# ExaScience/bpmf

Hardware: AMD Instinct MI355X
Metric: user+item column samples/sec per Gibbs iter; test RMSE vs reference (higher is better)
Workload: dtype f64

## Files before the change

### bpmf_amd/csrc/kernels.h

```cpp
#pragma once
#include <hip/hip_runtime.h>
#include <stdint.h>

#include "philox.h"
#include "args.h"

namespace bpmf {

typedef double d4 __attribute__((ext_vector_type(4)));

__device__ __forceinline__ d4 mfma16(double a, double b, d4 c)
{
    return __builtin_amdgcn_mfma_f64_16x16x4f64(a, b, c, 0, 0, 0);
}

__device__ __forceinline__ double mfma44(double a, double b, double c)
{
    return __builtin_amdgcn_mfma_f64_4x4x4f64(a, b, c, 0, 0, 0);
}

template <int K>
struct Rot44 {
    static constexpr int NT = K / 16;
    __host__ __device__ static constexpr int nrot(int TI, int TJ) { return TI == TJ ? 3 : 4; }
    __host__ __device__ static constexpr int aoff(int TI, int TJ)
    {
        int n = 0;
        for (int a = 0; a < NT; ++a)
            for (int b = a; b < NT; ++b) {
                if (a == TI && b == TJ) return n;
                n += nrot(a, b);
            }
        return n;
    }
    static constexpr int NACC = aoff(NT - 1, NT - 1) + 3;
};

template <int D>
__device__ __forceinline__ double quad_rot(double x)
{
    constexpr int CTRL = 0x120 + (16 - 4 * D);
    const long long v = __builtin_bit_cast(long long, x);
    const int lo = __builtin_amdgcn_update_dpp(0, (int)v, CTRL, 0xF, 0xF, true);
    const int hi = __builtin_amdgcn_update_dpp(0, (int)(v >> 32), CTRL, 0xF, 0xF, true);
    return __builtin_bit_cast(double, ((long long)hi << 32) | (unsigned int)lo);
}

template <int K>
__device__ __forceinline__ void rot44_contract(const double (&yy)[K / 16], double (&C)[Rot44<K>::NACC])
{
    using G = Rot44<K>;
    constexpr int NT = K / 16;
    double rot[NT][3];
#pragma unroll
    for (int t = 0; t < NT; ++t) {
        rot[t][0] = yy[t];
        rot[t][1] = quad_rot<1>(yy[t]);
        rot[t][2] = quad_rot<2>(yy[t]);
    }
#pragma unroll
    for (int TI = 0; TI < NT; ++TI)
#pragma unroll
        for (int TJ = TI; TJ < NT; ++TJ)
#pragma unroll
            for (int d = 0; d < G::nrot(TI, TJ); ++d) {
                if (d < 3) C[G::aoff(TI, TJ) + d] = mfma44(yy[TI], rot[TJ][d], C[G::aoff(TI, TJ) + d]);
                else C[G::aoff(TI, TJ) + d] = mfma44(rot[TI][1], yy[TJ], C[G::aoff(TI, TJ) + d]);
            }
}

template <int K, typename Sink>
__device__ __forceinline__ void rot44_images(const double (&C)[Rot44<K>::NACC], double *buf0, double *buf1, int lane, Sink &&sink)
{
    using G = Rot44<K>;
    constexpr int NT = G::NT;
    const int i = lane >> 4, b = (lane >> 2) & 3, j = lane & 3;
    int tix = 0;
#pragma unroll
    for (int TI = 0; TI < NT; ++TI)
#pragma unroll
        for (int TJ = TI; TJ < NT; ++TJ, ++tix) {
            double *img = (tix & 1) ? buf1 : buf0;
#pragma unroll
            for (int d = 0; d < G::nrot(TI, TJ); ++d) {
                const int row = d < 3 ? 4 * b + i : 4 * ((b + 1) & 3) + i, col = d < 3 ? 4 * ((b + d) & 3) + j : 4 * b + j;
                const double v = C[G::aoff(TI, TJ) + d];
                img[row * 16 + col] = v;
                if (TI == TJ && d > 0) img[col * 16 + row] = v;
            }
            __syncthreads();
#pragma unroll
            for (int m = 0; m < 4; ++m) sink(tix, TI, TJ, m, img[(4 * m + i) * 16 + (lane & 15)]);
            __syncthreads();
        }
}

__device__ __forceinline__ double rsqrt_nr(double d)
{
    const double y0 = __builtin_amdgcn_rsq(d);
    const double e = fma(-d, y0 * y0, 1.0);
    const double q = e * fma(0.375, e, 0.5);
    return fma(y0, q, y0);
}

__device__ __forceinline__ double gbcast(double v, int base_bytes, int off)
{
    const int lo = __builtin_amdgcn_ds_bpermute(base_bytes + 4 * off, __double2loint(v));
    const int hi = __builtin_amdgcn_ds_bpermute(base_bytes + 4 * off, __double2hiint(v));
    return __hiloint2double(hi, lo);
}

__device__ __forceinline__ double bcast(double v, int src)
{
    const int lo = __builtin_amdgcn_readlane(__double2loint(v), src);
    const int hi = __builtin_amdgcn_readlane(__double2hiint(v), src);
    return __hiloint2double(hi, lo);
}


__device__ __forceinline__ double polar_r2(double x, double y)
{
#pragma clang fp contract(off)
    return x * x + y * y;
}

__device__ __forceinline__ uint32_t sample_counter(int64_t idx, int ktrue, uint32_t iter_plus_1)
{
    return (uint32_t)((uint64_t)(idx + 1) * (uint64_t)ktrue * (uint64_t)iter_plus_1);
}

#define BPMF_RLX_SYSTEM_ __ATOMIC_RELAXED, __HIP_MEMORY_SCOPE_SYSTEM
enum { BPMF_TMO_GATE = 1, BPMF_TMO_PARAMS = 2, BPMF_TMO_STATS = 3 };
__device__ __forceinline__ void flag_timeout(unsigned long long *tmo, unsigned long long what)
{
    if (tmo) __hip_atomic_store(tmo, what, BPMF_RLX_SYSTEM_);
}

__device__ __forceinline__ void wait_params(const SampleArgs &a)
{
    if (a.gate_flag == nullptr) return;
    const unsigned long long t0 = wall_clock64();
    const unsigned long long limit = a.wait_ticks + (a.wait_ticks >> 1);
    while ((unsigned)__builtin_amdgcn_readfirstlane((int)__hip_atomic_load(a.gate_flag, __ATOMIC_RELAXED, __HIP_MEMORY_SCOPE_AGENT)) != a.gate_want) {
        __builtin_amdgcn_s_sleep(8);
        if (wall_clock64() - t0 > limit) {
            if (threadIdx.x == 0) flag_timeout(a.tmo, BPMF_TMO_PARAMS);
            break;
        }
    }
    asm volatile("" ::: "memory");
}

#ifndef BPMF_PROFILING
#define BPMF_PROFILING 0
#endif
constexpr bool kProfiling = BPMF_PROFILING != 0;
__device__ __forceinline__ uint32_t ablate_bits(const SampleArgs &a)
{
    if constexpr (kProfiling) return a.ablate;
    else return 0u;
}

__device__ __forceinline__ void stamp(const SampleArgs &a, int w, int slot)
{
    if constexpr (!kProfiling) {
        __builtin_amdgcn_sched_barrier(0);
        return;
    }
    if (a.stamps == nullptr || threadIdx.x != 0) return;
    const int probe = (w == 0) ? 0 : ((w == a.nwork / 2) ? 1 : -1);
    if (probe >= 0 && slot < 64) a.stamps[probe * 64 + slot] = wall_clock64();
}

__device__ __forceinline__ int rank_below(unsigned long long m)
{
    return (int)__builtin_amdgcn_mbcnt_hi((unsigned)(m >> 32), __builtin_amdgcn_mbcnt_lo((unsigned)m, 0u));
}

template <int NMAX>
__device__ __forceinline__ void draw_normals(uint32_t counter, int n, double *out_lds, int lane, int pad_to = 0)
{
    for (int i = n + lane; i < pad_to; i += 64) out_lds[i] = 0.0;
    int produced = 0;
    uint32_t base = 0;
    while (produced < n) {
        const Philox4 b = stream_block(counter, base + (uint32_t)lane);
        const double x = 2.0 * canonical53(b.w[3], b.w[2]) - 1.0;
        const double y = 2.0 * canonical53(b.w[1], b.w[0]) - 1.0;
        const double r2 = polar_r2(x, y);
        const bool acc = !(r2 > 1.0 || r2 == 0.0);
        const unsigned long long m = __ballot(acc);
        const int rank = produced + rank_below(m);
        if (acc && rank < n) {
            out_lds[rank] = y * polar_mult(r2);
        }
        produced += __popcll(m);
        base += 64u;
    }
}

template <int NMAX>
__device__ __forceinline__ void draw_normals_deferred(uint32_t counter, int n, double *out_lds, double *r2_lds, int lane, int pad_to = 0)
{
    for (int i = n + lane; i < pad_to; i += 64) out_lds[i] = 0.0;
    int produced = 0;
    uint32_t base = 0;
    while (produced < n) {
        const Philox4 b = stream_block(counter, base + (uint32_t)lane);
        const double x = 2.0 * canonical53(b.w[3], b.w[2]) - 1.0;
        const double y = 2.0 * canonical53(b.w[1], b.w[0]) - 1.0;
        const double r2 = polar_r2(x, y);
        const bool acc = !(r2 > 1.0 || r2 == 0.0);
        const unsigned long long m = __ballot(acc);
        const int rank = produced + rank_below(m);
        if (acc && rank < n) { out_lds[rank] = y; r2_lds[rank] = r2; }
        produced += __popcll(m);
        base += 64u;
    }
    for (int i = lane; i < n; i += 64) {
        const double r2 = r2_lds[i];
        out_lds[i] = out_lds[i] * polar_mult(r2);
    }
}

template <int NMAX>
__device__ __forceinline__ void draw_normals_pair(uint32_t counterA, uint32_t counterB, int n, double *outA, double *outB,
                                                  double *r2A, double *r2B, int lane, int pad_to = 0)
{
    for (int i = n + lane; i < pad_to; i += 64) { outA[i] = 0.0; outB[i] = 0.0; }
    auto attempt = [&](uint32_t counter, uint32_t block, double &y, double &r2) -> bool {
        const Philox4 b = stream_block(counter, block);
        const double x = 2.0 * canonical53(b.w[3], b.w[2]) - 1.0;
        y = 2.0 * canonical53(b.w[1], b.w[0]) - 1.0;
        r2 = polar_r2(x, y);
        return !(r2 > 1.0 || r2 == 0.0);
    };
    int prodA, prodB;
    {
        double y, r2;
        bool acc = attempt(counterA, (uint32_t)lane, y, r2);
        unsigned long long m = __ballot(acc);
        int rank = rank_below(m);
        if (acc && rank < n) { outA[rank] = y; r2A[rank] = r2; }
        prodA = __popcll(m);
        acc = attempt(counterB, (uint32_t)lane, y, r2);
        m = __ballot(acc);
        rank = rank_below(m);
        if (acc && rank < n) { outB[rank] = y; r2B[rank] = r2; }
        prodB = __popcll(m);
    }
    const bool hi = lane >= 32;
    const int l32 = lane & 31;
    uint32_t base = 64u;
    while (prodA < n || prodB < n) {
        double y, r2;
        const bool acc = attempt(hi ? counterB : counterA, base + (uint32_t)l32, y, r2);
        const unsigned long long m = __ballot(acc);
        const unsigned mA = (unsigned)m, mB = (unsigned)(m >> 32);
        const int rank = hi ? prodB + (int)__builtin_amdgcn_mbcnt_hi(mB, 0u) : prodA + (int)__builtin_amdgcn_mbcnt_lo(mA, 0u);
        if (acc && rank < n) { (hi ? outB : outA)[rank] = y; (hi ? r2B : r2A)[rank] = r2; }
        prodA += __popc(mA); prodB += __popc(mB);
        base += 32u;
    }
    for (int i = lane; i < n; i += 64) {
        const double ra = r2A[i], rb = r2B[i];
        outA[i] = outA[i] * polar_mult(ra);
        outB[i] = outB[i] * polar_mult(rb);
    }
}

template <int K>
__device__ __forceinline__ void gram_chunk(const int32_t *__restrict__ rowidx, const double *__restrict__ vals, int len,
                                           const double *__restrict__ other, const double *__restrict__ zero_row, double mean, double alpha,
                                           d4 (&acc)[Geo<K>::NTRI], double (&r)[Geo<K>::NT], int lane, int rowmask = -1)
{
    constexpr int NT = Geo<K>::NT;
    const int kq = lane >> 4, li = lane & 15;
    int ri_n = (0 + lane < len) ? rowidx[lane] : -1;
    double wv_n = (0 + lane < len) ? (vals[lane] - mean) * alpha : 0.0;
    for (int b = 0; b < len; b += 64) {
        const int ri = ri_n;
        const double wv = wv_n;
        if (b + 64 < len) {
            const int q = b + 64 + lane;
            ri_n = (q < len) ? rowidx[q] : -1;
            wv_n = (q < len) ? (vals[q] - mean) * alpha : 0.0;
        }
        const int nsteps = (len - b >= 64) ? 16 : (len - b + 3) >> 2;
        double y[4][NT], w[4];
        auto gather = [&](int g, double (&yy)[4][NT], double (&ww)[4]) {
#pragma unroll
            for (int s = 0; s < 4; ++s) {
                const int src = (g * 4 + s) * 4 + kq;
                const int row = __shfl(ri, src);
                ww[s] = __shfl(wv, src);
                const double *col = (row >= 0) ? other + (size_t)(row & rowmask) * K : zero_row;
#pragma unroll
                for (int t = 0; t < NT; ++t) yy[s][t] = col[(t * 16 + li < K) ? t * 16 + li : 0];
            }
        };
        gather(0, y, w);
#pragma unroll
        for (int g = 0; g < 4; ++g) {
            if (g * 4 >= nsteps) break;
            double yn[4][NT], wn[4];
            const bool more = (g + 1) * 4 < nsteps;
            if (g < 3 && more) gather(g + 1, yn, wn);
#pragma unroll
            for (int s = 0; s < 4; ++s) {
#pragma unroll
                for (int t = 0; t < NT; ++t) r[t] = fma(y[s][t], w[s], r[t]);
                int tri = 0;
#pragma unroll
                for (int I = 0; I < NT; ++I)
#pragma unroll
                    for (int J = I; J < NT; ++J, ++tri) acc[tri] = mfma16(y[s][I], y[s][J], acc[tri]);
            }
            if (g < 3 && more) {
#pragma unroll
                for (int s = 0; s < 4; ++s) {
                    w[s] = wn[s];
#pragma unroll
                    for (int t = 0; t < NT; ++t) y[s][t] = yn[s][t];
                }
            }
        }
    }
#pragma unroll
    for (int t = 0; t < NT; ++t) {
        r[t] += __shfl_xor(r[t], 16);
        r[t] += __shfl_xor(r[t], 32);
    }
}

template <int CTRL>
__device__ __forceinline__ double row_ror_add(double x)
{
    const long long v = __builtin_bit_cast(long long, x);
    const int lo = (int)v, hi = (int)(v >> 32);
    const int rlo = __builtin_amdgcn_update_dpp(0, lo, CTRL, 0xF, 0xF, true);
    const int rhi = __builtin_amdgcn_update_dpp(0, hi, CTRL, 0xF, 0xF, true);
    const long long rv = ((long long)rhi << 32) | (unsigned int)rlo;
    return x + __builtin_bit_cast(double, rv);
}

struct IdxBlock { int ri; double v; int base; };
__device__ __forceinline__ IdxBlock load_idx_block(const int32_t *__restrict__ rowidx, const double *__restrict__ vals, int base, int lane, int len,
                                                   const double *__restrict__ safe)
{
    IdxBlock r;
    const int q = base + lane;
    const int32_t *pr = (q < len) ? rowidx + q : reinterpret_cast<const int32_t *>(safe);
    const double *pv = (q < len) ? vals + q : safe;
    r.ri = *pr;
    r.v = *pv;
    r.base = base;
    return r;
}

template <int K>
__device__ __forceinline__ void gram_chunk44(const int32_t *__restrict__ rowidx, const double *__restrict__ vals, int len,
                                             const double *__restrict__ other, const double *__restrict__ zero_row,
                                             double mean, double alpha, IdxBlock cur, IdxBlock nxt,
                                             double (&acc)[Geo44<K>::NB], double (&rr)[Geo44<K>::NG], int lane, int rowmask = -1)
{
    using G = Geo44<K>;
    constexpr int NG = G::NG, NL = G::NL;
    typedef double dd2 __attribute__((ext_vector_type(2)));
    const int slot = lane >> 2, x = lane & 3;
    auto gather = [&](const IdxBlock &ib, int gg, dd2 (&yy)[NL], double &ww) {
        const int src = gg * 16 + slot;
        const int row = __shfl(ib.ri, src);
        ww = (__shfl(ib.v, src) - mean) * alpha;
        const double *base = (ib.base + src < len) ? other + (size_t)(row & rowmask) * K : zero_row;
        const dd2 *p = reinterpret_cast<const dd2 *>(base + 2 * x);
#pragma unroll
        for (int h = 0; h < NL; ++h) yy[h] = p[4 * h];
    };
    auto contract = [&](const dd2 (&yy)[NL], double ww) {
        double R[NG];
#pragma unroll
        for (int h = 0; h < NL; ++h) { R[2 * h] = yy[h].x; R[2 * h + 1] = yy[h].y; }
#pragma unroll
        for (int g = 0; g < NG; ++g) rr[g] = fma(R[g], ww, rr[g]);
        int blk = 0;
#pragma unroll
        for (int g = 0; g < NG; ++g)
#pragma unroll
            for (int g2 = g; g2 < NG; ++g2, ++blk) acc[blk] = mfma44(R[g], R[g2], acc[blk]);
    };
    if (len <= 0) return;
    dd2 yA[NL], yB[NL];
    double wA, wB = 0.0;
    gather(cur, 0, yA, wA);
    int b0 = 0;
    for (; b0 + 64 < len; b0 += 64) {
        const IdxBlock nn = load_idx_block(rowidx, vals, b0 + 128, lane, len, zero_row);
        gather(cur, 1, yB, wB);
        contract(yA, wA);
        gather(cur, 2, yA, wA);
        contract(yB, wB);
        gather(cur, 3, yB, wB);
        contract(yA, wA);
        gather(nxt, 0, yA, wA);
        contract(yB, wB);
        cur = nxt;
        nxt = nn;
    }
    const int ng = (len - b0 + 15) >> 4;
    if (ng > 1) gather(cur, 1, yB, wB);
    contract(yA, wA);
    if (ng > 1) {
        if (ng > 2) gather(cur, 2, yA, wA);
        contract(yB, wB);
        if (ng > 2) {
            if (ng > 3) gather(cur, 3, yB, wB);
            contract(yA, wA);
            if (ng > 3) contract(yB, wB);
        }
    }
}

template <int K>
__device__ __forceinline__ void assemble44(double (&acc)[Geo44<K>::NB], double (&rr)[Geo44<K>::NG], double *sA, double *sb,
                                           int LD, int lane)
{
    using G = Geo44<K>;
    constexpr int NG = G::NG;
    static_assert(NG % 2 == 0, "block rows are written in pairs");
    const int i = lane >> 4, b = (lane >> 2) & 3, j = lane & 3;
    auto blk = [](int g, int g2) constexpr { return g * NG - (g * (g - 1)) / 2 + (g2 - g); };
    double *up = sA + (2 * i) * LD + 2 * j;
    double *lo = sA + (2 * j) * LD + 2 * i;
#pragma unroll
    for (int g = 0; g < NG; g += 2) {
#pragma unroll
        for (int t = blk(g, g); t < blk(g + 1, NG - 1) + 1; ++t) {
            const double v = row_ror_add<0x128>(acc[t]);
            acc[t] = row_ror_add<0x124>(v);
        }
        if (b == 0) {
            up[G::idx(g + 1, 0) * LD + G::idx(g + 1, 0)] = acc[blk(g + 1, g + 1)];
#pragma unroll
            for (int g2 = g; g2 < NG; g2 += 2) {
                double2 v; v.x = acc[blk(g, g2)]; v.y = acc[blk(g, g2 + 1)];
                *reinterpret_cast<double2 *>(&up[G::idx(g, 0) * LD + G::idx(g2, 0)]) = v;
                if (g2 > g) {
                    double2 w; w.x = acc[blk(g + 1, g2)]; w.y = acc[blk(g + 1, g2 + 1)];
                    *reinterpret_cast<double2 *>(&up[G::idx(g + 1, 0) * LD + G::idx(g2, 0)]) = w;
                }
            }
        } else if (b == 1) {
            lo[G::idx(g + 1, 0) * LD + G::idx(g, 0)] = acc[blk(g, g + 1)];
#pragma unroll
            for (int g2 = g + 2; g2 < NG; ++g2) {
                double2 v; v.x = acc[blk(g, g2)]; v.y = acc[blk(g + 1, g2)];
                *reinterpret_cast<double2 *>(&lo[G::idx(g2, 0) * LD + G::idx(g, 0)]) = v;
            }
        }
    }
#pragma unroll
    for (int g = 0; g < NG; ++g) {
        double v = row_ror_add<0x128>(rr[g]);
        v = row_ror_add<0x124>(v);
        v += __shfl_xor(v, 16);
        v += __shfl_xor(v, 32);
        if (lane < 4) sb[G::idx(g, lane)] = v;
    }
}

template <int K>
__device__ __forceinline__ void deposit_column(const SampleArgs &a, int64_t idx, const d4 (&acc)[Geo<K>::NTRI],
                                               const double (&r)[Geo<K>::NT], double *lds, int slot, int lane)
{
    using G = Geo<K>;
    constexpr int NT = G::NT;
    const int kq = lane >> 4, li = lane & 15;
    double *sL = lds + slot * G::SLOT, *sY = sL + G::PLEN, *sZ = sY + K;

    draw_normals<K>(sample_counter(idx, a.ktrue, a.iter_plus_1), a.ktrue, sZ, lane, K);
    const double *LF = a.prop_lambda ? a.prop_lambda + (size_t)(idx - a.col_from) * K * K : a.LambdaF;

    int tri = 0;
#pragma unroll
    for (int I = 0; I < NT; ++I)
#pragma unroll
        for (int J = I; J < NT; ++J, ++tri)
#pragma unroll
            for (int reg = 0; reg < 4; ++reg) {
                const int gi = I * 16 + kq + 4 * reg, gj = J * 16 + li;
                const int row = (I == J) ? gi : gj, col = (I == J) ? gj : gi;
                if (row < K && col <= row)
                    sL[tri_off(row) + col] = (a.diag_only && row != col) ? 0.0 : fma(a.alpha, acc[tri][reg], LF[row + col * K]);
            }
    if (kq == 0) {
#pragma unroll
        for (int t = 0; t < NT; ++t)
            if (t * 16 + li < K) {
                double lm = a.Lmu[t * 16 + li];
                if (a.prop_lambda) {
                    lm = 0.0;
                    for (int j = 0; j < K; ++j) lm = fma(LF[t * 16 + li + j * K], a.mu[j], lm);
                }
                sY[t * 16 + li] = lm + r[t];
            }
    }
    if (lane == 0) reinterpret_cast<long long *>(lds + G::C * G::SLOT)[slot] = idx;
}

template <int K>
struct Pivot { double dinv0, dinv1, l10; };

template <int K>
__device__ __forceinline__ Pivot<K> factor_block(double pa, double pb, double pc)
{
    Pivot<K> v;
    v.dinv0 = rsqrt_nr(pa);
    const double rdet = rsqrt_nr(fma(pa, pc, -(pb * pb)));
    v.dinv1 = rdet * (pa * v.dinv0);
    v.l10 = pb * v.dinv0;
    return v;
}

template <int K>
__device__ __forceinline__ void finish_slots(const SampleArgs &a, double *lds, int nfilled, int lane_in)
{
    using G = Geo<K>;
    constexpr int NP = G::NP;
    int lane = lane_in;
    asm volatile("" : "+v"(lane));
    const int c = lane / K, i = lane % K;
    double *sL = lds + c * G::SLOT, *sY = sL + G::PLEN, *sZ = sY + K;
    double *myrow = sL + tri_off(i);
    const int gbase = 4 * (c * K);
    __syncthreads();

    double row[K + 1];
#pragma unroll
    for (int j = 0; j < K; j += 2) {
        const double2 g = *reinterpret_cast<const double2 *>(&myrow[j]);
        row[j] = g.x;
        row[j + 1] = g.y;
    }
    row[K] = sY[i];
    const double zi = sZ[i];
    Pivot<K> pv = factor_block<K>(sL[0], sL[tri_off(1)], sL[tri_off(1) + 1]);
    __syncthreads();

#pragma unroll
    for (int p = 0; p < NP; ++p) {
        const int k = 2 * p;
        double2 lp;
        lp.x = row[k] * pv.dinv0;
        lp.y = fma(-lp.x, pv.l10, row[k + 1]) * pv.dinv1;
        if (i >= k) *reinterpret_cast<double2 *>(&myrow[k]) = lp;

        double na = 0.0, nb = 0.0, nc = 0.0;
        if (p + 1 < NP) {
            na = gbcast(row[k + 2], gbase, k + 2);
            nb = gbcast(row[k + 2], gbase, k + 3);
            nc = gbcast(row[k + 3], gbase, k + 3);
        }
        const double rb0 = gbcast(row[K], gbase, k), rb1 = gbcast(row[K], gbase, k + 1);
        __syncthreads();
        const double2 L = *reinterpret_cast<const double2 *>(&myrow[k]);
        Pivot<K> pn = pv;
        if (p + 1 < NP) {
            const double2 l0 = *reinterpret_cast<const double2 *>(&sL[tri_off(k + 2) + k]);
            const double2 l1 = *reinterpret_cast<const double2 *>(&sL[tri_off(k + 3) + k]);
            const double pa = fma(-l0.y, l0.y, fma(-l0.x, l0.x, na));
            const double pb = fma(-l1.y, l0.y, fma(-l1.x, l0.x, nb));
            const double pc = fma(-l1.y, l1.y, fma(-l1.x, l1.x, nc));
            pn = factor_block<K>(pa, pb, pc);
        }
        const double yk = rb0 * pv.dinv0;
        const double yk1 = fma(-pv.l10, yk, rb1) * pv.dinv1;
        if (i == 0) *reinterpret_cast<double2 *>(&sY[k]) = double2{yk, yk1};
        row[K] = fma(-L.y, yk1, fma(-L.x, yk, row[K]));
#pragma unroll
        for (int j = k + 2; j < K; ++j) {
            const double2 A = *reinterpret_cast<const double2 *>(&sL[tri_off(j) + k]);
            row[j] = fma(-L.y, A.y, fma(-L.x, A.x, row[j]));
        }
#pragma unroll
        for (int m = k + 2; m < K + 1; ++m) asm volatile("" : "+v"(row[m]));
        pv = pn;
    }
    __syncthreads();

    double bi = sY[i] + zi;
    const double my_dinv = 1.0 / myrow[i];
    constexpr int BB = K < 8 ? K : 8;
#pragma unroll
    for (int kb = K - BB; kb >= 0; kb -= BB) {
        double lv[BB];
#pragma unroll
        for (int t = 0; t < BB; ++t) lv[t] = sL[tri_off(kb + t) + i];
#pragma unroll
        for (int t = BB - 1; t >= 0; --t) {
            const int k = kb + t;
            if (k == 0) continue;
            const double xk = gbcast(bi * my_dinv, gbase, k);
            bi = (i < k) ? fma(-lv[t], xk, bi) : bi;
        }
    }
    const double xi = bi * my_dinv;

    if (c < nfilled) {
        const long long idx = reinterpret_cast<const long long *>(lds + G::C * G::SLOT)[c];
        a.items[(size_t)idx * K + i] = xi;
        if (!(fabs(xi) <= 1.79769313486231570815e+308)) atomicMin(a.fail, (unsigned long long)idx);
    }
    __syncthreads();
}

#define BPMF_RLX_AGENT __ATOMIC_RELAXED, __HIP_MEMORY_SCOPE_AGENT

template <int K>
struct Geo1 {
    static constexpr int S = (64 / K < K / 2) ? 64 / K : K / 2;
    static constexpr int NP = K / 2;
    static constexpr int QN = NP / S;
    static constexpr int M = 2 * QN;
    static constexpr int FLD = K + 2;
    static constexpr bool PACKED = K == 64;
    __host__ __device__ static constexpr int roff_c(int j) { return (j & 1) ? ((j + 1) * (j + 1)) / 2 : (j * (j + 2)) / 2; }
    static constexpr int AWORDS = PACKED ? roff_c(K) : K * FLD;
    static constexpr int LANES = K * S;
    static constexpr int LDS_WORDS = AWORDS + 4 * K + 2;
    static constexpr int WPS = K == 32 ? 3 : (K < 32 ? 4 : 2);
};

template <int K, typename Assemble>
__device__ __forceinline__ void finish_single(const SampleArgs &a, int col_local, double *lds, int lane_in, bool have_z,
                                              Assemble &&assemble)
{
    int lane = lane_in;
    using G = Geo1<K>;
    constexpr int LD = G::FLD, S = G::S, NP = G::NP, QN = G::QN, M = G::M;
    asm volatile("" : "+v"(lane));
    double *sA = lds, *sb = lds + G::AWORDS, *sz = sb + K, *sdummy = sz + K, *szero = sdummy + 2 * K;
    auto roff = [](int j) -> int {
        if constexpr (G::PACKED) return (j & 1) ? ((j + 1) * (j + 1)) >> 1 : (j * (j + 2)) >> 1;
        else return j * G::FLD;
    };
    const int64_t idx = a.col_from + col_local;

    if (!have_z) draw_normals<K>(sample_counter(idx, a.ktrue, a.iter_plus_1), a.ktrue, sz, lane, K);

    const int l = lane & (G::LANES - 1);
    const int h = l / K, i = l % K;
    const double *LF = a.prop_lambda ? a.prop_lambda + (size_t)col_local * K * K : a.LambdaF;
    constexpr bool PRELOAD = K <= 32;
    double lf[PRELOAD ? M : 2];
    if constexpr (PRELOAD) {
#pragma unroll
        for (int q = 0; q < QN; ++q) {
            const int j = 2 * (q * S + h);
            lf[2 * q] = LF[i + j * K];
            lf[2 * q + 1] = LF[i + (j + 1) * K];
        }
    }
    double lmu = a.Lmu[i];
    if (a.prop_lambda) {
        lmu = 0.0;
        for (int j = 0; j < K; ++j) lmu = fma(LF[i + j * K], a.mu[j], lmu);
    }

    assemble(sA, sb, LD, lane);
    if (lane < 2) szero[lane] = 0.0;
    __syncthreads();

    double row[M + 2];
#pragma unroll
    for (int q = 0; q < QN; ++q) {
        double2 g;
        if constexpr (G::PACKED) {
            const int j = 2 * (q * S + h);
            g.x = sA[(j <= i) ? roff(i) + j : roff(j) + i];
            g.y = sA[(j + 1 <= i) ? roff(i) + j + 1 : roff(j + 1) + i];
        } else {
            g = *reinterpret_cast<const double2 *>(&sA[i * LD + 2 * (q * S + h)]);
        }
        if constexpr (PRELOAD) {
            row[2 * q] = fma(a.alpha, g.x, lf[2 * q]);
            row[2 * q + 1] = fma(a.alpha, g.y, lf[2 * q + 1]);
        } else {
            const int j = 2 * (q * S + h);
            row[2 * q] = fma(a.alpha, g.x, LF[i + j * K]);
            row[2 * q + 1] = fma(a.alpha, g.y, LF[i + (j + 1) * K]);
        }
    }
    if (a.diag_only) {
#pragma unroll
        for (int q = 0; q < QN; ++q) {
            const int j = 2 * (q * S + h);
            row[2 * q] = (j == i) ? row[2 * q] : 0.0;
            row[2 * q + 1] = (j + 1 == i) ? row[2 * q + 1] : 0.0;
        }
    }
    row[M] = (h == 0) ? lmu + sb[i] : 0.0;
    row[M + 1] = 0.0;
    const double zi = sz[i];
    double yi = 0.0;
    __syncthreads();

#pragma unroll
    for (int p = 0; p < NP; ++p) {
        const int hk = p % S, qk = p / S, k = 2 * p;
        const int src0 = hk * K + k, src1 = src0 + 1;
        const double pa = bcast(row[2 * qk], src0);
        const double pb = bcast(row[2 * qk], src1);
        const double pc = bcast(row[2 * qk + 1], src1);
        const double bk = bcast(row[M], k), bk1 = bcast(row[M], k + 1);
        const double dinv0 = rsqrt_nr(pa);
        const double rdet = rsqrt_nr(fma(pa, pc, -(pb * pb)));
        const double dinv1 = rdet * (pa * dinv0);
        const double l10 = pb * dinv0;
        const double yk = bk * dinv0;
        const double yk1 = fma(-l10, yk, bk1) * dinv1;
        yi = (i == k) ? yk : yi;
        yi = (i == k + 1) ? yk1 : yi;
        double2 lp;
        lp.x = row[2 * qk] * dinv0;
        lp.y = fma(-lp.x, l10, row[2 * qk + 1]) * dinv1;
        double *dst = (h == hk && (!G::PACKED || i >= k)) ? &sA[roff(i) + k] : &sdummy[2 * i];
        *reinterpret_cast<double2 *>(dst) = lp;
        __syncthreads();
        const double2 L = *reinterpret_cast<const double2 *>((!G::PACKED || i >= k) ? &sA[roff(i) + k] : szero);
        row[M] = fma(-L.y, yk1, fma(-L.x, yk, row[M]));
        if constexpr (S > 1) {
            const int j0 = 2 * (qk * S + h);
            const double2 A0 = *reinterpret_cast<const double2 *>(&sA[roff(j0) + k]);
            const double2 A1 = *reinterpret_cast<const double2 *>(&sA[roff(j0 + 1) + k]);
            const double u0 = fma(-L.y, A0.y, fma(-L.x, A0.x, row[2 * qk]));
            const double u1 = fma(-L.y, A1.y, fma(-L.x, A1.x, row[2 * qk + 1]));
            row[2 * qk] = (h > hk) ? u0 : row[2 * qk];
            row[2 * qk + 1] = (h > hk) ? u1 : row[2 * qk + 1];
        }
#pragma unroll
        for (int q = qk + 1; q < QN; ++q) {
            const int j0 = 2 * (q * S + h);
            const double2 A0 = *reinterpret_cast<const double2 *>(&sA[roff(j0) + k]);
            const double2 A1 = *reinterpret_cast<const double2 *>(&sA[roff(j0 + 1) + k]);
            row[2 * q] = fma(-L.y, A0.y, fma(-L.x, A0.x, row[2 * q]));
            row[2 * q + 1] = fma(-L.y, A1.y, fma(-L.x, A1.x, row[2 * q + 1]));
        }
#pragma unroll
        for (int m = 2 * qk; m < M + 1; ++m) asm volatile("" : "+v"(row[m]));
    }

    double bi = yi + zi;
    const double my_dinv = 1.0 / sA[roff(i) + i];
    constexpr int BB = K < 8 ? K : 8;
#pragma unroll
    for (int kb = K - BB; kb >= 0; kb -= BB) {
        double lv[BB];
#pragma unroll
        for (int t = 0; t < BB; ++t) lv[t] = *((i < kb + t) ? &sA[roff(kb + t) + i] : szero);
#pragma unroll
        for (int t = BB - 1; t >= 0; --t) {
            const int k = kb + t;
            if (k == 0) continue;
            const double xk = bcast(bi * my_dinv, k);
            bi = fma(-lv[t], xk, bi);
        }
    }
    const double xi = bi * my_dinv;

    if (lane < K) a.items[(size_t)idx * K + lane] = xi;
    const bool bad = !(fabs(xi) <= 1.79769313486231570815e+308);
    if (__any(bad) && lane == 0) atomicMin(a.fail, (unsigned long long)idx);
}

template <int K>
__device__ __forceinline__ void colstats_body(int w, const double *__restrict__ items, int64_t c0, int64_t c1, int nwaves,
                                              double *partials, const unsigned long long *__restrict__ fail_in,
                                              double *__restrict__ out, unsigned *ticket, unsigned *flag, unsigned seq,
                                              unsigned long long *tmo, unsigned long long wait_ticks, double *img);
__device__ __forceinline__ void gate_stage_body(int block, int nblocks, const unsigned *gate_host, unsigned want, const double *src_host,
                                                double *__restrict__ dst, int n, unsigned *dflag, unsigned dval,
                                                unsigned long long *tmo, unsigned long long wait_ticks);

template <int K>
__global__ __launch_bounds__(64, Geo1<K>::WPS) void k_sample1(SampleArgs a, FusedArgs f)
{
    __shared__ __attribute__((aligned(16))) double lds[Geo1<K>::LDS_WORDS];
    const int lane = threadIdx.x;
    int bid = blockIdx.x;
    if (f.gate_host) {
        if (bid == 0) { gate_stage_body(0, 1, f.gate_host, f.gate_want, f.src_host, f.dst, f.n, f.dflag, f.dval, a.tmo, a.wait_ticks); return; }
        --bid;
    }
    if (bid < f.nstat) {
        colstats_body<K>(bid, f.st_items, f.st_c0, f.st_c1, f.nstat, f.st_partials, f.st_fail, f.st_out, f.st_ticket, f.st_flag, f.st_seq,
                         f.st_tmo, a.wait_ticks, lds);
        return;
    }
    const int w = bid - f.nstat;
    const int col = a.wi_col[w];
    const int64_t p0 = a.wi_p0[w];
    const int len = a.wi_len[w];
    const int mc = a.wi_mc[w];

    const int glen = (ablate_bits(a) & 2u) ? 0 : len;
    const IdxBlock ib0 = load_idx_block(a.rowidx + p0, a.vals + p0, 0, lane, glen, a.zero_row);
    const IdxBlock ib1 = load_idx_block(a.rowidx + p0, a.vals + p0, 64, lane, glen, a.zero_row);

    if (mc < 0 && !(ablate_bits(a) & 1u))
        draw_normals<K>(sample_counter(a.col_from + col, a.ktrue, a.iter_plus_1), a.ktrue, lds + Geo1<K>::AWORDS + K, lane, K);

    static_assert(K <= 32, "k_sample1: K <= 32 (K = 64 runs the slab form, K = 128 the workgroup form)");
    {
        using G4 = Geo44<K>;
        constexpr int NB = G4::NB, NG = G4::NG, PART = G4::PART;
        double acc[NB], rr[NG];
#pragma unroll
        for (int t = 0; t < NB; ++t) acc[t] = 0.0;
#pragma unroll
        for (int t = 0; t < NG; ++t) rr[t] = 0.0;
        gram_chunk44<K>(a.rowidx + p0, a.vals + p0, glen, a.other_items, a.zero_row, a.mean_rating, a.alpha, ib0, ib1, acc, rr, lane,
                        (ablate_bits(a) & 4u) ? 63 : -1);
        if (ablate_bits(a) & 1u) {
            double v = rr[0];
#pragma unroll
            for (int t = 0; t < NB; ++t) v += acc[t];
            if (mc < 0 && lane < K) a.items[(size_t)(a.col_from + col) * K + lane] = v;
            return;
        }
        if (mc >= 0) {
            const int nch = a.mc_nchunks[mc];
            double *pbase = a.partials + (size_t)a.mc_slot0[mc] * PART;
            double *p = pbase + (size_t)a.wi_chunk[w] * PART;
#pragma unroll
            for (int t = 0; t < NB; ++t) __hip_atomic_store(&p[t * 64 + lane], acc[t], BPMF_RLX_AGENT);
#pragma unroll
            for (int t = 0; t < NG; ++t) __hip_atomic_store(&p[(NB + t) * 64 + lane], rr[t], BPMF_RLX_AGENT);
            asm volatile("s_waitcnt vmcnt(0)" ::: "memory");
            unsigned t = 0;
            if (lane == 0) t = __hip_atomic_fetch_add(&a.mc_count[mc], 1u, BPMF_RLX_AGENT);
            t = __builtin_amdgcn_readfirstlane(t);
            if ((int)t != nch - 1) return;
            if (lane == 0) __hip_atomic_store(&a.mc_count[mc], 0u, BPMF_RLX_AGENT);
#pragma unroll
            for (int t2 = 0; t2 < NB; ++t2) acc[t2] = 0.0;
#pragma unroll
            for (int t2 = 0; t2 < NG; ++t2) rr[t2] = 0.0;
            for (int ch = 0; ch < nch; ++ch) {
                const double *pc = pbase + (size_t)ch * PART;
                double tmp[NB + NG];
#pragma unroll
                for (int t2 = 0; t2 < NB + NG; ++t2) tmp[t2] = __hip_atomic_load(&pc[t2 * 64 + lane], BPMF_RLX_AGENT);
#pragma unroll
                for (int t2 = 0; t2 < NB; ++t2) acc[t2] += tmp[t2];
#pragma unroll
                for (int t2 = 0; t2 < NG; ++t2) rr[t2] += tmp[NB + t2];
            }
        }
        wait_params(a);
        finish_single<K>(a, col, lds, lane, mc < 0,
                         [&](double *sA, double *sb, int LD, int ln) { assemble44<K>(acc, rr, sA, sb, LD, ln); });
    }
}

#define BPMF_RLX_SYSTEM __ATOMIC_RELAXED, __HIP_MEMORY_SCOPE_SYSTEM
__device__ __forceinline__ void publish_when_last(unsigned *ticket, unsigned nblocks, unsigned *flag_host, unsigned seq,
                                                  unsigned *rearm = nullptr, unsigned *rearm2 = nullptr)
{
    asm volatile("s_waitcnt vmcnt(0)" ::: "memory");
    __syncthreads();
    if (threadIdx.x == 0) {
        const unsigned t = __hip_atomic_fetch_add(ticket, 1u, BPMF_RLX_AGENT);
        if (t == nblocks - 1) {
            __hip_atomic_store(ticket, 0u, BPMF_RLX_AGENT);
            if (rearm) __hip_atomic_store(rearm, 0u, BPMF_RLX_AGENT);
            if (rearm2) __hip_atomic_store(rearm2, 0u, BPMF_RLX_AGENT);
            __hip_atomic_store(flag_host, seq, BPMF_RLX_SYSTEM);
        }
    }
}

template <int K>
constexpr bool kColstatsRot = (K == 64);

template <int K>
__device__ __forceinline__ void colstats_accumulate(const double *__restrict__ items, int64_t b, int64_t e,
                                                    d4 (&acc)[Geo<K>::NTRI], double (&r)[Geo<K>::NT], int lane, double *img,
                                                    const int32_t *__restrict__ list = nullptr, int64_t c0 = 0)
{
    constexpr int NT = Geo<K>::NT;
    constexpr bool ROT = kColstatsRot<K>;
    const int kq = lane >> 4, li = lane & 15;
    double C[ROT ? Rot44<K>::NACC : 1];
#pragma unroll
    for (int t = 0; t < (ROT ? Rot44<K>::NACC : 1); ++t) C[t] = 0.0;
#pragma unroll
    for (int t = 0; t < Geo<K>::NTRI; ++t) acc[t] = d4{0.0, 0.0, 0.0, 0.0};
#pragma unroll
    for (int t = 0; t < NT; ++t) r[t] = 0.0;
    double yn[2][NT];
    int64_t idn[2];
    auto ids = [&](int64_t c, int64_t (&id)[2]) {
#pragma unroll
        for (int s = 0; s < 2; ++s) {
            const int64_t pos = (c + s * 4 + kq < e) ? c + s * 4 + kq : b;
            id[s] = list ? c0 + (int64_t)list[pos] : pos;
        }
    };
    auto fetch = [&](const int64_t (&id)[2], double (&yy)[2][NT]) {
#pragma unroll
        for (int s = 0; s < 2; ++s) {
            const double *x = items + (size_t)id[s] * K;
#pragma unroll
            for (int t = 0; t < NT; ++t) yy[s][t] = x[(t * 16 + li < K) ? t * 16 + li : 0];
        }
    };
    if (b < e) {
        int64_t id0[2];
        ids(b, id0);
        fetch(id0, yn);
        ids((b + 8 < e) ? b + 8 : b, idn);
    }
    for (int64_t c = b; c < e; c += 8) {
        double y[2][NT];
#pragma unroll
        for (int s = 0; s < 2; ++s) {
            const bool ok = c + s * 4 + kq < e;
#pragma unroll
            for (int t = 0; t < NT; ++t) y[s][t] = (ok && (t * 16 + li < K)) ? yn[s][t] : 0.0;
        }
        fetch(idn, yn);
        ids((c + 16 < e) ? c + 16 : b, idn);
#pragma unroll
        for (int s = 0; s < 2; ++s) {
#pragma unroll
            for (int t = 0; t < NT; ++t) r[t] += y[s][t];
            if constexpr (ROT) {
                rot44_contract<K>(y[s], C);
            } else {
                int tri = 0;
#pragma unroll
                for (int I = 0; I < NT; ++I)
#pragma unroll
                    for (int J = I; J < NT; ++J, ++tri) acc[tri] = mfma16(y[s][I], y[s][J], acc[tri]);
            }
        }
    }
    if constexpr (ROT) rot44_images<K>(C, img, img + 256, lane, [&](int tix, int, int, int m, double v) { acc[tix][m] = v; });
#pragma unroll
    for (int t = 0; t < NT; ++t) {
        r[t] += __shfl_xor(r[t], 16);
        r[t] += __shfl_xor(r[t], 32);
    }
}

template <int K>
__device__ __forceinline__ void colstats_body(int w, const double *__restrict__ items, int64_t c0, int64_t c1, int nwaves,
                                              double *partials, const unsigned long long *__restrict__ fail_in,
                                              double *__restrict__ out, unsigned *ticket, unsigned *flag, unsigned seq,
                                              unsigned long long *tmo, unsigned long long wait_ticks, double *img)
{
    constexpr int NT = Geo<K>::NT, NTRI = Geo<K>::NTRI, PART = Geo<K>::PART;
    constexpr int NSUMS = blob::res_sums(K), NSLICE = (NSUMS + 15) / 16, FAILD = blob::res_failD(K), FAIL = blob::res_fail(K);
    const int lane = threadIdx.x;
    const int64_t n = c1 - c0;
    const int64_t per = (((n + nwaves - 1) / nwaves) + 3) & ~(int64_t)3;
    const int64_t b = c0 + w * per;
    const int64_t e = (b + per < c1) ? b + per : c1;

    {
        d4 acc[NTRI];
        double r[NT];
        colstats_accumulate<K>(items, b, e, acc, r, lane, img);
        double *p = partials + (size_t)w * PART;
#pragma unroll
        for (int t = 0; t < NTRI; ++t)
#pragma unroll
            for (int reg = 0; reg < 4; ++reg) __hip_atomic_store(&p[(t * 4 + reg) * 64 + lane], acc[t][reg], BPMF_RLX_AGENT);
        if (lane < 16) {
#pragma unroll
            for (int t = 0; t < NT; ++t) __hip_atomic_store(&p[NTRI * 256 + t * 16 + lane], r[t], BPMF_RLX_AGENT);
        }
    }

    const int nfin = nwaves < NSLICE ? nwaves : NSLICE;
    asm volatile("s_waitcnt vmcnt(0)" ::: "memory");
    unsigned tk = 0;
    if (lane == 0) tk = __hip_atomic_fetch_add(ticket, 1u, BPMF_RLX_AGENT);
    tk = __builtin_amdgcn_readfirstlane(tk);
    if ((int)tk < nwaves - nfin) return;
    const int f = (int)tk - (nwaves - nfin);
    if (lane == 0) {
        const unsigned long long t0 = wall_clock64();
        while (__hip_atomic_load(ticket, BPMF_RLX_AGENT) < (unsigned)nwaves) {
            __builtin_amdgcn_s_sleep(1);
            if (wait_ticks && wall_clock64() - t0 > wait_ticks) { flag_timeout(tmo, BPMF_TMO_STATS); break; }
        }
    }
    __syncthreads();

    const int o = lane & 15, grp = lane >> 4;
    for (int slice = f; slice < NSLICE; slice += nfin) {
        const int eo = slice * 16 + o;
        double s = 0.0;
        if (eo < NSUMS) {
            int off;
            if (eo < K * K) {
                int i = eo % K, j = eo / K;
                if (i > j) { const int t = i; i = j; j = t; }
                const int I = i >> 4, J = j >> 4;
                const int tri = I * NT - (I * (I - 1)) / 2 + (J - I);
                const int ii = i & 15, jj = j & 15;
                off = (tri * 4 + (ii >> 2)) * 64 + (ii & 3) * 16 + jj;
            } else {
                off = NTRI * 256 + (eo - K * K);
            }
            const int pw = (nwaves + 3) >> 2;
            const int w0 = grp * pw, w1 = (w0 + pw < nwaves) ? w0 + pw : nwaves;
            double acc[16];
#pragma unroll
            for (int u = 0; u < 16; ++u) acc[u] = 0.0;
            for (int ww = w0; ww < w1; ww += 16) {
                double v[16];
#pragma unroll
                for (int u = 0; u < 16; ++u)
                    v[u] = __hip_atomic_load(&partials[(size_t)((ww + u < w1) ? ww + u : w0) * PART + off], BPMF_RLX_AGENT);
#pragma unroll
                for (int u = 0; u < 16; ++u) acc[u] += (ww + u < w1) ? v[u] : 0.0;
            }
#pragma unroll
            for (int h = 8; h >= 1; h >>= 1)
#pragma unroll
                for (int u = 0; u < h; ++u) acc[u] += acc[u + h];
            s = acc[0];
        }
        s += __shfl_xor(s, 16);
        s += __shfl_xor(s, 32);
        if (grp == 0 && eo < NSUMS) __hip_atomic_store(&out[eo], s, BPMF_RLX_SYSTEM);
    }
    if (f == 0 && lane == 0) {
        const unsigned long long fw = __hip_atomic_load(fail_in, BPMF_RLX_AGENT);
        __hip_atomic_store(&out[FAILD], (fw == ~0ull) ? 0.0 : (double)(fw + 1ull), BPMF_RLX_SYSTEM);
        __hip_atomic_store(&reinterpret_cast<unsigned long long *>(out)[FAIL], fw, BPMF_RLX_SYSTEM);
    }
    publish_when_last(ticket + 1, (unsigned)nfin, flag, seq, ticket);
}

template <int K>
__global__ __launch_bounds__(64) void k_colstats(const double *__restrict__ items, int64_t c0, int64_t c1, int nwaves,
                                                 double *partials, const unsigned long long *__restrict__ fail_in,
                                                 double *__restrict__ out, unsigned *ticket, unsigned *flag, unsigned seq,
                                                 unsigned long long *tmo, unsigned long long wait_ticks)
{
    __shared__ double img[kColstatsRot<K> ? 512 : 1];
    colstats_body<K>((int)blockIdx.x, items, c0, c1, nwaves, partials, fail_in, out, ticket, flag, seq, tmo, wait_ticks, img);
}

template <int K>
__global__ __launch_bounds__(256) void k_colstats_wg(const double *__restrict__ items, int64_t c0, int64_t c1, int nwg,
                                                    double *partials, const unsigned long long *__restrict__ fail_in,
                                                    double *__restrict__ out, unsigned *ticket, unsigned *flag, unsigned seq,
                                                    unsigned long long *tmo, unsigned long long wait_ticks,
                                                    const int32_t *__restrict__ list, int part0, int ntot, int finish)
{
    constexpr int NT = Geo<K>::NT, NTRI = Geo<K>::NTRI, PART = Geo<K>::PART, NBLK = (PART + 63) / 64, FAILD = blob::res_failD(K), FAIL = blob::res_fail(K);
    __shared__ double red[PART];
    __shared__ double fin[4][64];
    __shared__ unsigned stk;
    const int tid = threadIdx.x, wave = tid >> 6, lane = tid & 63;
    const int64_t n = c1 - c0;
    const int nvw = nwg * 4, vw = (int)blockIdx.x * 4 + wave;
    const int64_t per = (((n + nvw - 1) / nvw) + 3) & ~(int64_t)3;
    const int64_t b = c0 + vw * per;
    const int64_t e = (b + per < c1) ? b + per : c1;
// ... 299 lines not shown
```

Measured before the change: 100.9 million.

## Replace Cholesky with block LDL-style elimination and 2x2-blocked backward solve

```diff
diff --git a/bpmf_amd/csrc/kernels.h b/bpmf_amd/csrc/kernels.h
--- a/bpmf_amd/csrc/kernels.h
+++ b/bpmf_amd/csrc/kernels.h
@@ -101,6 +101,13 @@
     const double e = fma(-d, y0 * y0, 1.0);
     const double q = e * fma(0.375, e, 0.5);
     return fma(y0, q, y0);
+}
+
+__device__ __forceinline__ double rcp_nr(double d)
+{
+    const double y0 = __builtin_amdgcn_rcp(d);
+    const double e = fma(-d, y0, 1.0);
+    return fma(y0, fma(e, e, e), y0);
 }
 
 __device__ __forceinline__ double gbcast(double v, int base_bytes, int off)
@@ -639,17 +646,15 @@
     using G = Geo1<K>;
     constexpr int LD = G::FLD, S = G::S, NP = G::NP, QN = G::QN, M = G::M;
     asm volatile("" : "+v"(lane));
-    double *sA = lds, *sb = lds + G::AWORDS, *sz = sb + K, *sdummy = sz + K, *szero = sdummy + 2 * K;
-    auto roff = [](int j) -> int {
-        if constexpr (G::PACKED) return (j & 1) ? ((j + 1) * (j + 1)) >> 1 : (j * (j + 2)) >> 1;
-        else return j * G::FLD;
-    };
+    static_assert(!G::PACKED, "finish_single keeps full rows of LD words in LDS (K <= 32)");
+    double *sA = lds, *sb = lds + G::AWORDS, *sz = sb + K, *sdummy = sz + K;
+    auto roff = [](int j) -> int { return j * G::FLD; };
     const int64_t idx = a.col_from + col_local;
 
     if (!have_z) draw_normals<K>(sample_counter(idx, a.ktrue, a.iter_plus_1), a.ktrue, sz, lane, K);
 
-    const int l = lane & (G::LANES - 1);
-    const int h = l / K, i = l % K;
+    int l = lane & (G::LANES - 1);
+    int h = l / K, i = l % K;
     const double *LF = a.prop_lambda ? a.prop_lambda + (size_t)col_local * K * K : a.LambdaF;
     constexpr bool PRELOAD = K <= 32;
     double lf[PRELOAD ? M : 2];
@@ -667,21 +672,16 @@
         for (int j = 0; j < K; ++j) lmu = fma(LF[i + j * K], a.mu[j], lmu);
     }
 
+    asm volatile("" : "+v"(lane));
+    l = lane & (G::LANES - 1);
+    h = l / K, i = l % K;
     assemble(sA, sb, LD, lane);
-    if (lane < 2) szero[lane] = 0.0;
     __syncthreads();
 
     double row[M + 2];
 #pragma unroll
     for (int q = 0; q < QN; ++q) {
-        double2 g;
-        if constexpr (G::PACKED) {
-            const int j = 2 * (q * S + h);
-            g.x = sA[(j <= i) ? roff(i) + j : roff(j) + i];
-            g.y = sA[(j + 1 <= i) ? roff(i) + j + 1 : roff(j + 1) + i];
-        } else {
-            g = *reinterpret_cast<const double2 *>(&sA[i * LD + 2 * (q * S + h)]);
-        }
+        const double2 g = *reinterpret_cast<const double2 *>(&sA[i * LD + 2 * (q * S + h)]);
         if constexpr (PRELOAD) {
             row[2 * q] = fma(a.alpha, g.x, lf[2 * q]);
             row[2 * q + 1] = fma(a.alpha, g.y, lf[2 * q + 1]);
@@ -701,40 +701,37 @@
     }
     row[M] = (h == 0) ? lmu + sb[i] : 0.0;
     row[M + 1] = 0.0;
-    const double zi = sz[i];
-    double yi = 0.0;
+    double ti = 0.0;
     __syncthreads();
 
 #pragma unroll
     for (int p = 0; p < NP; ++p) {
         const int hk = p % S, qk = p / S, k = 2 * p;
         const int src0 = hk * K + k, src1 = src0 + 1;
+        double2 rp;
+        rp.x = row[2 * qk];
+        rp.y = row[2 * qk + 1];
+        *reinterpret_cast<double2 *>((h == hk) ? &sA[roff(i) + k] : &sdummy[2 * i]) = rp;
         const double pa = bcast(row[2 * qk], src0);
         const double pb = bcast(row[2 * qk], src1);
         const double pc = bcast(row[2 * qk + 1], src1);
-        const double bk = bcast(row[M], k), bk1 = bcast(row[M], k + 1);
-        const double dinv0 = rsqrt_nr(pa);
-        const double rdet = rsqrt_nr(fma(pa, pc, -(pb * pb)));
-        const double dinv1 = rdet * (pa * dinv0);
-        const double l10 = pb * dinv0;
-        const double yk = bk * dinv0;
-        const double yk1 = fma(-l10, yk, bk1) * dinv1;
-        yi = (i == k) ? yk : yi;
-        yi = (i == k + 1) ? yk1 : yi;
-        double2 lp;
-        lp.x = row[2 * qk] * dinv0;
-        lp.y = fma(-lp.x, l10, row[2 * qk + 1]) * dinv1;
-        double *dst = (h == hk && (!G::PACKED || i >= k)) ? &sA[roff(i) + k] : &sdummy[2 * i];
-        *reinterpret_cast<double2 *>(dst) = lp;
+        const double tk = bcast(row[M], k), tk1 = bcast(row[M], k + 1);
+        const double ia = rcp_nr(pa);
+        const double idet = rcp_nr(fma(pa, pc, -(pb * pb)));
+        const double g = pb * ia, hh = pa * idet;
+        ti = (i >= k) ? row[M] : ti;
         __syncthreads();
-        const double2 L = *reinterpret_cast<const double2 *>((!G::PACKED || i >= k) ? &sA[roff(i) + k] : szero);
-        row[M] = fma(-L.y, yk1, fma(-L.x, yk, row[M]));
+        const double2 R = *reinterpret_cast<const double2 *>(&sA[roff(i) + k]);
+        double2 w;
+        w.y = fma(-g, R.x, R.y) * hh;
+        w.x = fma(-g, w.y, R.x * ia);
+        row[M] = fma(-w.y, tk1, fma(-w.x, tk, row[M]));
         if constexpr (S > 1) {
             const int j0 = 2 * (qk * S + h);
             const double2 A0 = *reinterpret_cast<const double2 *>(&sA[roff(j0) + k]);
             const double2 A1 = *reinterpret_cast<const double2 *>(&sA[roff(j0 + 1) + k]);
-            const double u0 = fma(-L.y, A0.y, fma(-L.x, A0.x, row[2 * qk]));
-            const double u1 = fma(-L.y, A1.y, fma(-L.x, A1.x, row[2 * qk + 1]));
+            const double u0 = fma(-w.y, A0.y, fma(-w.x, A0.x, row[2 * qk]));
+            const double u1 = fma(-w.y, A1.y, fma(-w.x, A1.x, row[2 * qk + 1]));
             row[2 * qk] = (h > hk) ? u0 : row[2 * qk];
             row[2 * qk + 1] = (h > hk) ? u1 : row[2 * qk + 1];
         }
@@ -743,33 +740,61 @@
             const int j0 = 2 * (q * S + h);
             const double2 A0 = *reinterpret_cast<const double2 *>(&sA[roff(j0) + k]);
             const double2 A1 = *reinterpret_cast<const double2 *>(&sA[roff(j0 + 1) + k]);
-            row[2 * q] = fma(-L.y, A0.y, fma(-L.x, A0.x, row[2 * q]));
-            row[2 * q + 1] = fma(-L.y, A1.y, fma(-L.x, A1.x, row[2 * q + 1]));
+            row[2 * q] = fma(-w.y, A0.y, fma(-w.x, A0.x, row[2 * q]));
+            row[2 * q + 1] = fma(-w.y, A1.y, fma(-w.x, A1.x, row[2 * q + 1]));
         }
 #pragma unroll
         for (int m = 2 * qk; m < M + 1; ++m) asm volatile("" : "+v"(row[m]));
     }
 
-    double bi = yi + zi;
-    const double my_dinv = 1.0 / sA[roff(i) + i];
-    constexpr int BB = K < 8 ? K : 8;
-#pragma unroll
-    for (int kb = K - BB; kb >= 0; kb -= BB) {
-        double lv[BB];
-#pragma unroll
-        for (int t = 0; t < BB; ++t) lv[t] = *((i < kb + t) ? &sA[roff(kb + t) + i] : szero);
-#pragma unroll
-        for (int t = BB - 1; t >= 0; --t) {
-            const int k = kb + t;
-            if (k == 0) continue;
-            const double xk = bcast(bi * my_dinv, k);
-            bi = fma(-lv[t], xk, bi);
-        }
-    }
-    const double xi = bi * my_dinv;
+    static_assert(2 * K >= LD + 2, "the zero rows of the backward solve live in the dummy slots");
+    const int ip = i >> 1;
+    double2 zero2;
+    zero2.x = zero2.y = 0.0;
+    *reinterpret_cast<double2 *>(&sdummy[0]) = zero2;
+    *reinterpret_cast<double2 *>(&sdummy[LD]) = zero2;
+    const double pa = sA[roff(2 * ip) + 2 * ip];
+    const double2 pbc = *reinterpret_cast<const double2 *>(&sA[roff(2 * ip + 1) + 2 * ip]);
+    const double2 zz = *reinterpret_cast<const double2 *>(&sz[2 * ip]);
+    __syncthreads();
+    const bool odd = i & 1;
+    const double d0 = rsqrt_nr(pa);
+    const double rdet = rsqrt_nr(fma(pa, pbc.y, -(pbc.x * pbc.x)));
+    const double d1 = rdet * (pa * d0);
+    const double idet = rdet * rdet;
+    const double u1 = zz.y * d1;
+    const double u0 = fma(-(pbc.x * d0), u1, zz.x) * d0;
+    const double cown = (odd ? pa : pbc.y) * idet, ccr = -(pbc.x * idet);
+    const double cx = odd ? ccr : cown, cy = odd ? cown : ccr;
+    const double tp = __hiloint2double(__builtin_amdgcn_update_dpp(0, __double2hiint(ti), 0xB1, 0xF, 0xF, true),
+                                       __builtin_amdgcn_update_dpp(0, __double2loint(ti), 0xB1, 0xF, 0xF, true));
+    const double base = fma(cown, ti, fma(ccr, tp, odd ? u1 : u0));
+    double sx = 0.0, sy = 0.0;
+    constexpr int NBB = NP < 4 ? NP : 4;
+#pragma unroll
+    for (int qb = NP - NBB; qb >= 0; qb -= NBB) {
+        double2 lv[2 * NBB];
+#pragma unroll
+        for (int t = 0; t < NBB; ++t) {
+            const double *src = (ip < qb + t) ? &sA[roff(2 * (qb + t)) + 2 * ip] : sdummy;
+            lv[2 * t] = *reinterpret_cast<const double2 *>(src);
+            lv[2 * t + 1] = *reinterpret_cast<const double2 *>(src + LD);
+        }
+#pragma unroll
+        for (int t = NBB - 1; t >= 0; --t) {
+            if (qb + t == 0) continue;
+            const double xc = fma(-cy, sy, fma(-cx, sx, base));
+            const double x1 = bcast(xc, 2 * (qb + t) + 1), x0 = bcast(xc, 2 * (qb + t));
+            sx = fma(lv[2 * t + 1].x, x1, sx);
+            sy = fma(lv[2 * t + 1].y, x1, sy);
+            sx = fma(lv[2 * t].x, x0, sx);
+            sy = fma(lv[2 * t].y, x0, sy);
+        }
+    }
+    const double xi = fma(-cy, sy, fma(-cx, sx, base));
 
     if (lane < K) a.items[(size_t)idx * K + lane] = xi;
-    const bool bad = !(fabs(xi) <= 1.79769313486231570815e+308);
+    const bool bad = lane < K && !(fabs(xi) <= 1.79769313486231570815e+308);
     if (__any(bad) && lane == 0) atomicMin(a.fail, (unsigned long long)idx);
 }
 
```

New measurement: 103.3 million (median of 5 runs). +2.3%, better.
